# createamind/Distributed-DRL

Measured on AMD Instinct MI355X. Metric: env-steps/s + learner updates/s, SAC1 LunarLanderContinuous-v2 @1/2/4/8 GPU, higher is better.
Workload: dtype f32

## Files before the change

### distributed-drl_amd/csrc/loop.hip

```cpp
#include "ddrl_common.h"

#include <cstdlib>
#include <cstring>
#include <vector>

int ddrl_sac1_internal_opt_sync(ddrl_sac1_t *h, void *stream);
int ddrl_sac1_internal_sample_into(ddrl_sac1_t *h, ddrl_replay_t *replay, int set, void *stream);

struct ddrl_loop {
    ddrl_sac1_t *learner;
    ddrl_replay_t *replay;
    int per_graph;
    uint32_t seed;
    float *buf[2][8];
    int batch;
    hipGraphExec_t exec;
    bool captured;
    int parity;
};

static int sample_into(ddrl_loop *h, int set, void *stream) {
    return ddrl_sac1_internal_sample_into(h->learner, h->replay, set, stream);
}

static int update_from(ddrl_loop *h, int set, void *stream) {
    float **b = h->buf[set];
    int rc = ddrl_sac1_fill_noise(h->learner, h->seed, stream);
    if (rc != DDRL_OK) return rc;
    return ddrl_sac1_step(h->learner, b[0], b[1], b[2], b[3], b[4], b[5], b[6], b[7], nullptr, nullptr, nullptr, nullptr, stream);
}

static int one_update(ddrl_loop *h, void *stream) {
    const int set = h->parity;
    h->parity ^= 1;
    int rc = sample_into(h, set, stream);
    if (rc != DDRL_OK) return rc;
    return update_from(h, set, stream);
}

static int grads_from(ddrl_loop *h, int set, void *stream) {
    float **b = h->buf[set];
    int rc = ddrl_sac1_fill_noise(h->learner, h->seed, stream);
    if (rc != DDRL_OK) return rc;
    return ddrl_sac1_compute_grads(h->learner, b[0], b[1], b[2], b[3], b[4], b[5], b[6], b[7], nullptr, nullptr, nullptr, nullptr,
                                   stream);
}

static int capture(ddrl_loop *h, hipStream_t main_s) {
    const char *fk = getenv("DDRL_LOOP_FORK");
    const int mode = !fk ? 0 : (strcmp(fk, "all") == 0 ? 2 : 1);
    hipStream_t side = nullptr;
    DDRL_HIP_CHECK(hipStreamCreateWithFlags(&side, hipStreamNonBlocking));
    const int n = h->per_graph;
    std::vector<hipEvent_t> e_smp(n + 1), e_upd(n + 1), e_grad(n + 1);
    hipEvent_t e_fork;
    DDRL_HIP_CHECK(hipEventCreateWithFlags(&e_fork, hipEventDisableTiming));
    for (int i = 0; i <= n; ++i) {
        DDRL_HIP_CHECK(hipEventCreateWithFlags(&e_smp[i], hipEventDisableTiming));
        DDRL_HIP_CHECK(hipEventCreateWithFlags(&e_upd[i], hipEventDisableTiming));
        DDRL_HIP_CHECK(hipEventCreateWithFlags(&e_grad[i], hipEventDisableTiming));
    }
    hipGraph_t graph = nullptr;
    int rc = ddrl_sac1_internal_opt_sync(h->learner, (void *)main_s);
    if (rc != DDRL_OK) return rc;
    DDRL_HIP_CHECK(hipStreamSynchronize(main_s));
    DDRL_HIP_CHECK(hipStreamBeginCapture(main_s, hipStreamCaptureModeThreadLocal));
    hipError_t e = hipSuccess;
#define HE(x) do { if (e == hipSuccess && rc == DDRL_OK) e = (x); } while (0)
#define RC(x) do { if (e == hipSuccess && rc == DDRL_OK) rc = (x); } while (0)
    if (mode == 0) {
        RC(sample_into(h, 0, (void *)main_s));
        for (int i = 0; i < n; ++i) {
            RC(ddrl_sac1_fill_noise(h->learner, h->seed, (void *)main_s));
            if (i + 1 < n) {
                RC(ddrl_sac1_step_and_sample(h->learner, i & 1, h->replay, (i + 1) & 1, (void *)main_s));
            } else {
                float **b = h->buf[i & 1];
                RC(ddrl_sac1_step(h->learner, b[0], b[1], b[2], b[3], b[4], b[5], b[6], b[7], nullptr, nullptr, nullptr, nullptr,
                                  (void *)main_s));
            }
        }
    } else if (mode == 2) {
        HE(hipEventRecord(e_fork, main_s));
        HE(hipStreamWaitEvent(side, e_fork, 0));
        for (int i = 0; i < n; ++i) {
            if (i >= 2) HE(hipStreamWaitEvent(side, e_upd[i - 2], 0));
            RC(sample_into(h, i & 1, (void *)side));
            HE(hipEventRecord(e_smp[i], side));
            HE(hipStreamWaitEvent(main_s, e_smp[i], 0));
            RC(update_from(h, i & 1, (void *)main_s));
            HE(hipEventRecord(e_upd[i], main_s));
        }
    } else {
        RC(sample_into(h, 0, (void *)main_s));
        for (int i = 0; i < n; ++i) {
            RC(grads_from(h, i & 1, (void *)main_s));
            if (i + 1 < n) {
                HE(hipEventRecord(e_grad[i], main_s));
                HE(hipStreamWaitEvent(side, e_grad[i], 0));
                RC(sample_into(h, (i + 1) & 1, (void *)side));
                HE(hipEventRecord(e_smp[i + 1], side));
            }
            RC(ddrl_sac1_apply_grads(h->learner, (void *)main_s));
            if (i + 1 < n) HE(hipStreamWaitEvent(main_s, e_smp[i + 1], 0));
        }
    }
    RC(ddrl_sac1_internal_opt_sync(h->learner, (void *)main_s));
#undef HE
#undef RC
    hipError_t e2 = hipStreamEndCapture(main_s, &graph);
    for (int i = 0; i <= n; ++i) { (void)hipEventDestroy(e_smp[i]); (void)hipEventDestroy(e_upd[i]); (void)hipEventDestroy(e_grad[i]); }
    (void)hipEventDestroy(e_fork);
    (void)hipStreamDestroy(side);
    if (rc != DDRL_OK) { if (graph) (void)hipGraphDestroy(graph); return rc; }
    if (e != hipSuccess || e2 != hipSuccess) {
        ddrl::set_error("graph capture failed: %s", hipGetErrorString(e != hipSuccess ? e : e2));
        if (graph) (void)hipGraphDestroy(graph);
        return DDRL_ERR_HIP;
    }
    DDRL_HIP_CHECK(hipGraphInstantiate(&h->exec, graph, nullptr, nullptr, 0));
    (void)hipGraphDestroy(graph);
    h->captured = true;
    return DDRL_OK;
}

extern "C" {

int ddrl_loop_create(ddrl_loop_t **out, ddrl_sac1_t *learner, ddrl_replay_t *replay, int32_t updates_per_graph,
                     uint32_t noise_seed) {
    DDRL_REQUIRE(out && learner && replay, "NULL pointer");
    DDRL_REQUIRE(updates_per_graph >= 0 && updates_per_graph <= 4096, "updates_per_graph must be in [0, 4096]");
    ddrl_loop *h = new ddrl_loop();
    h->learner = learner; h->replay = replay; h->per_graph = updates_per_graph; h->seed = noise_seed;
    h->exec = nullptr; h->captured = false; h->parity = 0;
    int rc = ddrl_sac1_input_buffers(learner, 0, h->buf[0]);
    if (rc == DDRL_OK) rc = ddrl_sac1_input_buffers(learner, 1, h->buf[1]);
    if (rc != DDRL_OK) { delete h; return rc; }
    h->batch = ddrl_sac1_batch(learner);
    *out = h;
    return DDRL_OK;
}

int ddrl_loop_destroy(ddrl_loop_t *h) {
    if (!h) return DDRL_OK;
    if (h->exec) (void)hipGraphExecDestroy(h->exec);
    delete h;
    return DDRL_OK;
}

int ddrl_loop_run(ddrl_loop_t *h, int64_t n_updates, void *stream) {
    DDRL_REQUIRE(h != nullptr && n_updates >= 0, "bad handle / n_updates");
    hipStream_t s = ddrl::as_stream(stream);
    int64_t left = n_updates;
    if (h->per_graph > 0 && left >= h->per_graph) {
        if (!h->captured) {
            int rc = one_update(h, stream);
            if (rc != DDRL_OK) return rc;
            left -= 1;
            hipStream_t cs = s, own = nullptr;
            if (cs == nullptr) {
                DDRL_HIP_CHECK(hipStreamCreateWithFlags(&own, hipStreamNonBlocking));
                DDRL_HIP_CHECK(hipDeviceSynchronize());
                cs = own;
            }
            rc = capture(h, cs);
            if (own) (void)hipStreamDestroy(own);
            if (rc != DDRL_OK) return rc;
        }
        if (left >= h->per_graph) {
            const int rc2 = ddrl_sac1_internal_opt_sync(h->learner, stream);
            if (rc2 != DDRL_OK) return rc2;
        }
        while (left >= h->per_graph) {
            DDRL_HIP_CHECK(hipGraphLaunch(h->exec, s));
            left -= h->per_graph;
        }
    }
    for (; left > 0; --left) {
        int rc = one_update(h, stream);
        if (rc != DDRL_OK) return rc;
    }
    return DDRL_OK;
}

}
```

Measured before the change: 44310.

## Run leftover updates through cached power-of-two CUDA-style graphs instead of eager steps

Result: no change. 44490, median of 6 (+0.4%).

```diff
diff --git a/distributed-drl_amd/csrc/loop.hip b/distributed-drl_amd/csrc/loop.hip
--- a/distributed-drl_amd/csrc/loop.hip
+++ b/distributed-drl_amd/csrc/loop.hip
@@ -15,7 +15,8 @@
     float *buf[2][8];
     int batch;
     hipGraphExec_t exec;
-    bool captured;
+    std::vector<hipGraphExec_t> rem;
+    bool primed;
     int parity;
 };
 
@@ -46,12 +47,11 @@
                                    stream);
 }
 
-static int capture(ddrl_loop *h, hipStream_t main_s) {
+static int capture(ddrl_loop *h, hipStream_t main_s, int n, hipGraphExec_t *out) {
     const char *fk = getenv("DDRL_LOOP_FORK");
     const int mode = !fk ? 0 : (strcmp(fk, "all") == 0 ? 2 : 1);
     hipStream_t side = nullptr;
     DDRL_HIP_CHECK(hipStreamCreateWithFlags(&side, hipStreamNonBlocking));
-    const int n = h->per_graph;
     std::vector<hipEvent_t> e_smp(n + 1), e_upd(n + 1), e_grad(n + 1);
     hipEvent_t e_fork;
     DDRL_HIP_CHECK(hipEventCreateWithFlags(&e_fork, hipEventDisableTiming));
@@ -63,7 +63,8 @@
     hipGraph_t graph = nullptr;
     int rc = ddrl_sac1_internal_opt_sync(h->learner, (void *)main_s);
     if (rc != DDRL_OK) return rc;
-    DDRL_HIP_CHECK(hipStreamSynchronize(main_s));
+    rc = ddrl_replay_counts(h->replay, nullptr, nullptr, nullptr, nullptr, (void *)main_s);
+    if (rc != DDRL_OK) return rc;
     DDRL_HIP_CHECK(hipStreamBeginCapture(main_s, hipStreamCaptureModeThreadLocal));
     hipError_t e = hipSuccess;
 #define HE(x) do { if (e == hipSuccess && rc == DDRL_OK) e = (x); } while (0)
@@ -118,9 +119,25 @@
         if (graph) (void)hipGraphDestroy(graph);
         return DDRL_ERR_HIP;
     }
-    DDRL_HIP_CHECK(hipGraphInstantiate(&h->exec, graph, nullptr, nullptr, 0));
+    const hipError_t e3 = hipGraphInstantiate(out, graph, nullptr, nullptr, 0);
     (void)hipGraphDestroy(graph);
-    h->captured = true;
+    DDRL_HIP_CHECK(e3);
+    return DDRL_OK;
+}
+
+static int replay(ddrl_loop *h, hipGraphExec_t *slot, int n, hipStream_t s) {
+    if (*slot == nullptr) {
+        hipStream_t cs = s, own = nullptr;
+        if (cs == nullptr) {
+            DDRL_HIP_CHECK(hipStreamCreateWithFlags(&own, hipStreamNonBlocking));
+            DDRL_HIP_CHECK(hipDeviceSynchronize());
+            cs = own;
+        }
+        const int rc = capture(h, cs, n, slot);
+        if (own) (void)hipStreamDestroy(own);
+        if (rc != DDRL_OK) return rc;
+    }
+    DDRL_HIP_CHECK(hipGraphLaunch(*slot, s));
     return DDRL_OK;
 }
 
@@ -132,7 +149,8 @@
     DDRL_REQUIRE(updates_per_graph >= 0 && updates_per_graph <= 4096, "updates_per_graph must be in [0, 4096]");
     ddrl_loop *h = new ddrl_loop();
     h->learner = learner; h->replay = replay; h->per_graph = updates_per_graph; h->seed = noise_seed;
-    h->exec = nullptr; h->captured = false; h->parity = 0;
+    h->exec = nullptr; h->primed = false; h->parity = 0;
+    for (int b = 0; (1 << b) < updates_per_graph; ++b) h->rem.push_back(nullptr);
     int rc = ddrl_sac1_input_buffers(learner, 0, h->buf[0]);
     if (rc == DDRL_OK) rc = ddrl_sac1_input_buffers(learner, 1, h->buf[1]);
     if (rc != DDRL_OK) { delete h; return rc; }
@@ -144,6 +162,7 @@
 int ddrl_loop_destroy(ddrl_loop_t *h) {
     if (!h) return DDRL_OK;
     if (h->exec) (void)hipGraphExecDestroy(h->exec);
+    for (hipGraphExec_t g : h->rem) if (g) (void)hipGraphExecDestroy(g);
     delete h;
     return DDRL_OK;
 }
@@ -152,29 +171,28 @@
     DDRL_REQUIRE(h != nullptr && n_updates >= 0, "bad handle / n_updates");
     hipStream_t s = ddrl::as_stream(stream);
     int64_t left = n_updates;
-    if (h->per_graph > 0 && left >= h->per_graph) {
-        if (!h->captured) {
+    if (h->per_graph > 0 && left > 0) {
+        if (!h->primed) {
             int rc = one_update(h, stream);
             if (rc != DDRL_OK) return rc;
+            h->primed = true;
             left -= 1;
-            hipStream_t cs = s, own = nullptr;
-            if (cs == nullptr) {
-                DDRL_HIP_CHECK(hipStreamCreateWithFlags(&own, hipStreamNonBlocking));
-                DDRL_HIP_CHECK(hipDeviceSynchronize());
-                cs = own;
-            }
-            rc = capture(h, cs);
-            if (own) (void)hipStreamDestroy(own);
-            if (rc != DDRL_OK) return rc;
-        }
-        if (left >= h->per_graph) {
-            const int rc2 = ddrl_sac1_internal_opt_sync(h->learner, stream);
-            if (rc2 != DDRL_OK) return rc2;
-        }
-        while (left >= h->per_graph) {
-            DDRL_HIP_CHECK(hipGraphLaunch(h->exec, s));
-            left -= h->per_graph;
-        }
+        }
+        if (left > 0) {
+            const int rc = ddrl_sac1_internal_opt_sync(h->learner, stream);
+            if (rc != DDRL_OK) return rc;
+        }
+        for (; left >= h->per_graph; left -= h->per_graph) {
+            const int rc = replay(h, &h->exec, h->per_graph, s);
+            if (rc != DDRL_OK) return rc;
+        }
+        for (int b = (int)h->rem.size() - 1; b >= 0; --b) {
+            if (!(left & ((int64_t)1 << b))) continue;
+            const int rc = replay(h, &h->rem[b], 1 << b, s);
+            if (rc != DDRL_OK) return rc;
+            left -= (int64_t)1 << b;
+        }
+        return DDRL_OK;
     }
     for (; left > 0; --left) {
         int rc = one_update(h, stream);
```
